# microsoft/XPretrain

Hardware: NVIDIA H100
Metric: video-text pairs/sec (12f x 224^2, 32 tok), CLIP-ViP ViT-B/16 fwd+InfoNCE+bwd (higher is better)
Workload: dtype bf16

## Files before the change

### xpretrain_b200/csrc/ptx.cuh

```cuda
#pragma once
#include <cuda.h>
#include <cuda_bf16.h>
#include <cuda_runtime.h>
#include <stdint.h>
#include <stdio.h>

namespace xp {

#ifndef XP_WAIT_TIMEOUT_CYCLES
#define XP_WAIT_TIMEOUT_CYCLES (8000000000ll)
#endif

__device__ __forceinline__ uint32_t smem_u32(const void* p) {
  return static_cast<uint32_t>(__cvta_generic_to_shared(p));
}
__device__ __forceinline__ int lane_id() { return threadIdx.x & 31; }

__device__ __forceinline__ void mbar_init(uint64_t* bar, uint32_t count) {
  asm volatile("mbarrier.init.shared::cta.b64 [%0], %1;" ::"r"(smem_u32(bar)), "r"(count) : "memory");
}
__device__ __forceinline__ void fence_barrier_init() {
  asm volatile("fence.mbarrier_init.release.cluster;" ::: "memory");
}
__device__ __forceinline__ void fence_proxy_async_smem() {
  asm volatile("fence.proxy.async.shared::cta;" ::: "memory");
}
__device__ __forceinline__ void mbar_arrive_expect_tx(uint64_t* bar, uint32_t bytes) {
  asm volatile("mbarrier.arrive.expect_tx.shared::cta.b64 _, [%0], %1;" ::"r"(smem_u32(bar)), "r"(bytes)
               : "memory");
}
__device__ __forceinline__ void mbar_arrive(uint64_t* bar) {
  asm volatile("mbarrier.arrive.shared::cta.b64 _, [%0];" ::"r"(smem_u32(bar)) : "memory");
}
__device__ __forceinline__ bool mbar_try_wait(uint64_t* bar, uint32_t parity) {
  uint32_t ok;
  asm volatile(
      "{\n"
      ".reg .pred p;\n"
      "mbarrier.try_wait.parity.shared::cta.b64 p, [%1], %2;\n"
      "selp.u32 %0, 1, 0, p;\n"
      "}\n"
      : "=r"(ok)
      : "r"(smem_u32(bar)), "r"(parity)
      : "memory");
  return ok != 0;
}
__device__ __forceinline__ void mbar_wait(uint64_t* bar, uint32_t parity) {
  if (mbar_try_wait(bar, parity)) return;
  long long t0 = clock64();
  while (!mbar_try_wait(bar, parity)) {
    if (clock64() - t0 > XP_WAIT_TIMEOUT_CYCLES) {
      printf("xpretrain_b200: mbarrier wait timeout (block %d thread %d parity %u)\n", blockIdx.x, threadIdx.x,
             parity);
      __trap();
    }
  }
}
__device__ __forceinline__ void mbar_wait_nocall(uint64_t* bar, uint32_t parity) {
  if (mbar_try_wait(bar, parity)) return;
  long long t0 = clock64();
  while (!mbar_try_wait(bar, parity)) {
    if (clock64() - t0 > XP_WAIT_TIMEOUT_CYCLES) __trap();
  }
}

__device__ __forceinline__ void tma_prefetch_desc(const CUtensorMap* m) {
  asm volatile("prefetch.tensormap [%0];" ::"l"(reinterpret_cast<uint64_t>(m)) : "memory");
}
__device__ __forceinline__ void tma_load_2d(void* smem_dst, const CUtensorMap* m, uint64_t* bar, int c0, int c1) {
  asm volatile(
      "cp.async.bulk.tensor.2d.shared::cluster.global.mbarrier::complete_tx::bytes [%0], [%1, {%3, %4}], [%2];"
      ::"r"(smem_u32(smem_dst)), "l"(reinterpret_cast<uint64_t>(m)), "r"(smem_u32(bar)), "r"(c0), "r"(c1)
      : "memory");
}
__device__ __forceinline__ void tma_load_3d(void* smem_dst, const CUtensorMap* m, uint64_t* bar, int c0, int c1,
                                            int c2) {
  asm volatile(
      "cp.async.bulk.tensor.3d.shared::cluster.global.mbarrier::complete_tx::bytes [%0], [%1, {%3, %4, %5}], [%2];"
      ::"r"(smem_u32(smem_dst)), "l"(reinterpret_cast<uint64_t>(m)), "r"(smem_u32(bar)), "r"(c0), "r"(c1), "r"(c2)
      : "memory");
}

__device__ __forceinline__ void tma_store_2d(const CUtensorMap* m, uint32_t smem_src, int c0, int c1) {
  asm volatile("cp.async.bulk.tensor.2d.global.shared::cta.bulk_group [%0, {%2, %3}], [%1];" ::"l"(
                   reinterpret_cast<uint64_t>(m)),
               "r"(smem_src), "r"(c0), "r"(c1)
               : "memory");
}
__device__ __forceinline__ void tma_store_commit() { asm volatile("cp.async.bulk.commit_group;" ::: "memory"); }
template <int N>
__device__ __forceinline__ void tma_store_wait_read() {
  asm volatile("cp.async.bulk.wait_group.read %0;" ::"n"(N) : "memory");
}

__device__ __forceinline__ void wgmma_fence() { asm volatile("wgmma.fence.sync.aligned;" ::: "memory"); }
__device__ __forceinline__ void wgmma_commit() { asm volatile("wgmma.commit_group.sync.aligned;" ::: "memory"); }
template <int N>
__device__ __forceinline__ void wgmma_wait() {
  asm volatile("wgmma.wait_group.sync.aligned %0;" ::"n"(N) : "memory");
}
template <int R>
__device__ __forceinline__ void wgmma_fence_regs(float (&d)[R]) {
#pragma unroll
  for (int i = 0; i < R; ++i) asm volatile("" : "+f"(d[i])::"memory");
}

template <int TA, int TB>
__device__ __forceinline__ void wgmma_m64n128k16_bf16(float (&d)[64], uint64_t adesc, uint64_t bdesc) {
  asm volatile(
      "wgmma.mma_async.sync.aligned.m64n128k16.f32.bf16.bf16 {"
      "%0, %1, %2, %3, %4, %5, %6, %7, %8, %9, %10, %11, %12, %13, %14, %15, "
      "%16, %17, %18, %19, %20, %21, %22, %23, %24, %25, %26, %27, %28, %29, %30, %31, "
      "%32, %33, %34, %35, %36, %37, %38, %39, %40, %41, %42, %43, %44, %45, %46, %47, "
      "%48, %49, %50, %51, %52, %53, %54, %55, %56, %57, %58, %59, %60, %61, %62, %63"
      "}, %64, %65, 1, 1, 1, %66, %67;"
      : "+f"(d[0]), "+f"(d[1]), "+f"(d[2]), "+f"(d[3]), "+f"(d[4]), "+f"(d[5]), "+f"(d[6]), "+f"(d[7]),
        "+f"(d[8]), "+f"(d[9]), "+f"(d[10]), "+f"(d[11]), "+f"(d[12]), "+f"(d[13]), "+f"(d[14]), "+f"(d[15]),
        "+f"(d[16]), "+f"(d[17]), "+f"(d[18]), "+f"(d[19]), "+f"(d[20]), "+f"(d[21]), "+f"(d[22]), "+f"(d[23]),
        "+f"(d[24]), "+f"(d[25]), "+f"(d[26]), "+f"(d[27]), "+f"(d[28]), "+f"(d[29]), "+f"(d[30]), "+f"(d[31]),
        "+f"(d[32]), "+f"(d[33]), "+f"(d[34]), "+f"(d[35]), "+f"(d[36]), "+f"(d[37]), "+f"(d[38]), "+f"(d[39]),
        "+f"(d[40]), "+f"(d[41]), "+f"(d[42]), "+f"(d[43]), "+f"(d[44]), "+f"(d[45]), "+f"(d[46]), "+f"(d[47]),
        "+f"(d[48]), "+f"(d[49]), "+f"(d[50]), "+f"(d[51]), "+f"(d[52]), "+f"(d[53]), "+f"(d[54]), "+f"(d[55]),
        "+f"(d[56]), "+f"(d[57]), "+f"(d[58]), "+f"(d[59]), "+f"(d[60]), "+f"(d[61]), "+f"(d[62]), "+f"(d[63])
      : "l"(adesc), "l"(bdesc), "n"(TA), "n"(TB));
}

template <int TA, int TB>
__device__ __forceinline__ void wgmma_m64n64k16_ss(float (&d)[32], uint64_t adesc, uint64_t bdesc) {
  asm volatile(
      "wgmma.mma_async.sync.aligned.m64n64k16.f32.bf16.bf16 {"
      "%0, %1, %2, %3, %4, %5, %6, %7, %8, %9, %10, %11, %12, %13, %14, %15, "
      "%16, %17, %18, %19, %20, %21, %22, %23, %24, %25, %26, %27, %28, %29, %30, %31"
      "}, %32, %33, 1, 1, 1, %34, %35;"
      : "+f"(d[0]), "+f"(d[1]), "+f"(d[2]), "+f"(d[3]), "+f"(d[4]), "+f"(d[5]), "+f"(d[6]), "+f"(d[7]),
        "+f"(d[8]), "+f"(d[9]), "+f"(d[10]), "+f"(d[11]), "+f"(d[12]), "+f"(d[13]), "+f"(d[14]), "+f"(d[15]),
        "+f"(d[16]), "+f"(d[17]), "+f"(d[18]), "+f"(d[19]), "+f"(d[20]), "+f"(d[21]), "+f"(d[22]), "+f"(d[23]),
        "+f"(d[24]), "+f"(d[25]), "+f"(d[26]), "+f"(d[27]), "+f"(d[28]), "+f"(d[29]), "+f"(d[30]), "+f"(d[31])
      : "l"(adesc), "l"(bdesc), "n"(TA), "n"(TB));
}
template <int TB>
__device__ __forceinline__ void wgmma_m64n64k16_rs(float (&d)[32], const uint32_t (&a)[4], uint64_t bdesc) {
  asm volatile(
      "wgmma.mma_async.sync.aligned.m64n64k16.f32.bf16.bf16 {"
      "%0, %1, %2, %3, %4, %5, %6, %7, %8, %9, %10, %11, %12, %13, %14, %15, "
      "%16, %17, %18, %19, %20, %21, %22, %23, %24, %25, %26, %27, %28, %29, %30, %31"
      "}, {%32, %33, %34, %35}, %36, 1, 1, 1, %37;"
      : "+f"(d[0]), "+f"(d[1]), "+f"(d[2]), "+f"(d[3]), "+f"(d[4]), "+f"(d[5]), "+f"(d[6]), "+f"(d[7]),
        "+f"(d[8]), "+f"(d[9]), "+f"(d[10]), "+f"(d[11]), "+f"(d[12]), "+f"(d[13]), "+f"(d[14]), "+f"(d[15]),
        "+f"(d[16]), "+f"(d[17]), "+f"(d[18]), "+f"(d[19]), "+f"(d[20]), "+f"(d[21]), "+f"(d[22]), "+f"(d[23]),
        "+f"(d[24]), "+f"(d[25]), "+f"(d[26]), "+f"(d[27]), "+f"(d[28]), "+f"(d[29]), "+f"(d[30]), "+f"(d[31])
      : "r"(a[0]), "r"(a[1]), "r"(a[2]), "r"(a[3]), "l"(bdesc), "n"(TB));
}

template <uint32_t N>
__device__ __forceinline__ void setmaxnreg_dec() {
  asm volatile("setmaxnreg.dec.sync.aligned.u32 %0;" ::"n"(N));
}
template <uint32_t N>
__device__ __forceinline__ void setmaxnreg_inc() {
  asm volatile("setmaxnreg.inc.sync.aligned.u32 %0;" ::"n"(N));
}
__device__ __forceinline__ void named_bar_sync(uint32_t id, uint32_t threads) {
  asm volatile("bar.sync %0, %1;" ::"r"(id), "r"(threads) : "memory");
}
__device__ __forceinline__ void named_bar_arrive(uint32_t id, uint32_t threads) {
  asm volatile("bar.arrive %0, %1;" ::"r"(id), "r"(threads) : "memory");
}

__device__ __forceinline__ uint64_t make_smem_desc_sw128(uint32_t smem_addr, uint32_t lbo_bytes,
                                                         uint32_t sbo_bytes) {
  uint64_t d = 0;
  d |= static_cast<uint64_t>((smem_addr & 0x3FFFF) >> 4);
  d |= static_cast<uint64_t>((lbo_bytes >> 4) & 0x3FFF) << 16;
  d |= static_cast<uint64_t>((sbo_bytes >> 4) & 0x3FFF) << 32;
  d |= static_cast<uint64_t>(1) << 62;
  return d;
}

__device__ __forceinline__ void quad_transpose(uint32_t (&v)[4]) {
  const int q = threadIdx.x & 3;
  uint32_t out[4];
  out[0] = out[1] = out[2] = out[3] = 0u;
#pragma unroll
  for (int t = 0; t < 4; ++t) {
    const int j = q ^ t;
    const uint32_t send = j == 0 ? v[0] : j == 1 ? v[1] : j == 2 ? v[2] : v[3];
    const uint32_t got = t == 0 ? send : __shfl_xor_sync(0xffffffffu, send, t);
#pragma unroll
    for (int c = 0; c < 4; ++c)
      if (c == j) out[c] = got;
  }
#pragma unroll
  for (int c = 0; c < 4; ++c) v[c] = out[c];
}

__device__ __forceinline__ uint32_t pack_bf16(float lo, float hi) {
  __nv_bfloat162 v = __floats2bfloat162_rn(lo, hi);
  return *reinterpret_cast<uint32_t*>(&v);
}
__device__ __forceinline__ float bf16_lo(uint32_t v) { return __uint_as_float(v << 16); }
__device__ __forceinline__ float bf16_hi(uint32_t v) { return __uint_as_float(v & 0xFFFF0000u); }

__device__ __forceinline__ float fast_sigmoid(float y) {
  float t;
  asm("tanh.approx.f32 %0, %1;" : "=f"(t) : "f"(0.5f * y));
  return fmaf(0.5f, t, 0.5f);
}
__device__ __forceinline__ float quick_gelu(float x) { return x * fast_sigmoid(1.702f * x); }
__device__ __forceinline__ float quick_gelu_grad(float x) {
  float y = 1.702f * x;
  y = y > 64.f ? 64.f : (y < -64.f ? -64.f : y);
  const float s = fast_sigmoid(y);
  return s * fmaf(y, 1.f - s, 1.f);
}

}
```

### xpretrain_b200/csrc/vip_attention.cu

```cuda
#include "../../include/xpretrain_b200.h"
#include "common.h"
#include "ptx.cuh"
#include "mma_frag.cuh"
#include "vip_attention.h"

namespace xp {

constexpr int SROWS = 256;
constexpr int GROW = 248;
constexpr int MAT_BYTES = SROWS * 128;
constexpr int TILE_BYTES = 64 * 128;
constexpr int ATT_THREADS = 256;

__device__ __forceinline__ bool row_valid(int r, const AttnDims& d) { return r < d.L || (r >= GROW && r < GROW + d.M); }
__device__ __forceinline__ bool row_global(int r) { return r >= GROW; }
__device__ __forceinline__ int row_seq(int r, const AttnDims& d) { return r >= GROW ? r - GROW : d.M + r; }
__device__ __forceinline__ bool tile_live(int k, const AttnDims& d) { return k == 3 || 64 * k < d.L; }

__device__ __forceinline__ uint64_t kdesc(uint32_t addr) { return make_smem_desc_sw128(addr, 16, 1024); }
__device__ __forceinline__ uint64_t mndesc(uint32_t addr) { return make_smem_desc_sw128(addr, 8192, 1024); }

template <int NMAT>
__device__ __forceinline__ void stage_rows(uint8_t* sm, uint64_t* bar, const CUtensorMap* const (&mapL)[NMAT],
                                           const CUtensorMap* const (&mapM)[NMAT], const int (&col)[NMAT], const AttnDims& d,
                                           int b, int t) {
  if (threadIdx.x == 0) {
    mbar_init(bar, 1);
    fence_barrier_init();
  }
  const uint32_t base = smem_u32(sm);
  for (int idx = threadIdx.x; idx < NMAT * SROWS * 8; idx += ATT_THREADS) {
    const int m = idx / (SROWS * 8), row = (idx >> 3) % SROWS;
    if (!row_valid(row, d)) st_shared_zero16(base + m * MAT_BYTES + row * 128 + (idx & 7) * 16);
  }
  fence_proxy_async_smem();
  __syncthreads();
  if (threadIdx.x == 0) {
    mbar_arrive_expect_tx(bar, NMAT * (d.L + d.M) * 128);
#pragma unroll
    for (int m = 0; m < NMAT; ++m) {
      tma_load_2d(sm + m * MAT_BYTES, mapL[m], bar, col[m], static_cast<int>(b * d.S + d.M + static_cast<long long>(t) * d.L));
      tma_load_2d(sm + m * MAT_BYTES + GROW * 128, mapM[m], bar, col[m], static_cast<int>(b * d.S));
    }
  }
  mbar_wait_nocall(bar, 0);
}

__device__ __forceinline__ void acc_to_afrag(const float (&x)[32], uint32_t (&a)[4][4]) {
#pragma unroll
  for (int ks = 0; ks < 4; ++ks) {
    a[ks][0] = pack_bf16(x[8 * ks + 0], x[8 * ks + 1]);
    a[ks][1] = pack_bf16(x[8 * ks + 2], x[8 * ks + 3]);
    a[ks][2] = pack_bf16(x[8 * ks + 4], x[8 * ks + 5]);
    a[ks][3] = pack_bf16(x[8 * ks + 6], x[8 * ks + 7]);
  }
}

__global__ void __launch_bounds__(ATT_THREADS, 2)
vip_attn_fwd_kernel(const __grid_constant__ CUtensorMap tmL, const __grid_constant__ CUtensorMap tmM,
                    __nv_bfloat16* __restrict__ out, float* __restrict__ lse, float* __restrict__ part, const AttnDims d) {
  extern __shared__ uint8_t smem_raw[];
  uint8_t* sm = smem_raw + (((smem_u32(smem_raw) + 1023u) & ~1023u) - smem_u32(smem_raw));
  uint64_t* bar = reinterpret_cast<uint64_t*>(sm + 3 * MAT_BYTES);
  const int t = blockIdx.x, h = blockIdx.y, b = blockIdx.z;
  {
    const CUtensorMap* const mL[3] = {&tmL, &tmL, &tmL};
    const CUtensorMap* const mM[3] = {&tmM, &tmM, &tmM};
    const int col[3] = {h * HD, d.C + h * HD, 2 * d.C + h * HD};
    stage_rows<3>(sm, bar, mL, mM, col, d, b, t);
  }
  const uint32_t sQ = smem_u32(sm), sK = sQ + MAT_BYTES, sV = sK + MAT_BYTES;
  const int wg = threadIdx.x >> 7, wq = (threadIdx.x >> 5) & 3, lane = threadIdx.x & 31;
  const bool mask_gg = (t != 0);

  for (int qt = wg; qt < 4; qt += 2) {
    if (!tile_live(qt, d)) continue;
    const int r_lo = qt * 64 + wq * 16 + (lane >> 2);
    const bool qg[2] = {row_global(r_lo), row_global(r_lo + 8)};
    float o[32];
#pragma unroll
    for (int i = 0; i < 32; ++i) o[i] = 0.f;
    float m_run[2] = {-INFINITY, -INFINITY}, l_run[2] = {0.f, 0.f};
#pragma unroll 1
    for (int kb = 0; kb < 4; ++kb) {
      if (!tile_live(kb, d)) continue;
      float s[32];
#pragma unroll
      for (int i = 0; i < 32; ++i) s[i] = 0.f;
      wgmma_fence_regs(s);
      wgmma_fence();
#pragma unroll
      for (int ks = 0; ks < 4; ++ks)
        wgmma_m64n64k16_ss<0, 0>(s, kdesc(sQ + qt * TILE_BYTES + ks * 32), kdesc(sK + kb * TILE_BYTES + ks * 32));
      wgmma_commit();
      wgmma_wait<0>();
      wgmma_fence_regs(s);
      float mx[2] = {-INFINITY, -INFINITY};
#pragma unroll
      for (int i = 0; i < 8; ++i)
#pragma unroll
        for (int e = 0; e < 4; ++e) {
          const int key = kb * 64 + i * 8 + (lane & 3) * 2 + (e & 1);
          const bool dead = !row_valid(key, d) || (mask_gg && qg[e >> 1] && row_global(key));
          if (dead) s[4 * i + e] = -INFINITY;
          mx[e >> 1] = fmaxf(mx[e >> 1], s[4 * i + e]);
        }
      float corr[2], mb[2];
#pragma unroll
      for (int r = 0; r < 2; ++r) {
        mx[r] = fmaxf(mx[r], __shfl_xor_sync(0xffffffffu, mx[r], 1));
        mx[r] = fmaxf(mx[r], __shfl_xor_sync(0xffffffffu, mx[r], 2));
        const float m_new = fmaxf(m_run[r], mx[r]);
        corr[r] = (m_new == -INFINITY) ? 1.f : fast_exp2((m_run[r] - m_new) * LOG2E);
        l_run[r] *= corr[r];
        m_run[r] = m_new;
        mb[r] = m_new == -INFINITY ? 0.f : m_new * LOG2E;
      }
#pragma unroll
      for (int i = 0; i < 8; ++i) {
        o[4 * i + 0] *= corr[0]; o[4 * i + 1] *= corr[0];
        o[4 * i + 2] *= corr[1]; o[4 * i + 3] *= corr[1];
      }
#pragma unroll
      for (int i = 0; i < 32; ++i) {
        const float pv = fast_exp2(fmaf(s[i], LOG2E, -mb[(i >> 1) & 1]));
        s[i] = pv;
        l_run[(i >> 1) & 1] += pv;
      }
      uint32_t ph[4][4], pl[4][4];
      acc_to_afrag(s, ph);
#pragma unroll
      for (int ks = 0; ks < 4; ++ks)
#pragma unroll
        for (int j = 0; j < 4; ++j)
          pl[ks][j] = pack_bf16(s[8 * ks + 2 * j] - bf16_lo(ph[ks][j]), s[8 * ks + 2 * j + 1] - bf16_hi(ph[ks][j]));
      wgmma_fence_regs(o);
      wgmma_fence();
#pragma unroll
      for (int ks = 0; ks < 4; ++ks) {
        const uint64_t vd = mndesc(sV + kb * TILE_BYTES + ks * 16 * 128);
        wgmma_m64n64k16_rs<1>(o, ph[ks], vd);
        wgmma_m64n64k16_rs<1>(o, pl[ks], vd);
      }
      wgmma_commit();
      wgmma_wait<0>();
      wgmma_fence_regs(o);
    }
#pragma unroll
    for (int r = 0; r < 2; ++r) {
      l_run[r] += __shfl_xor_sync(0xffffffffu, l_run[r], 1);
      l_run[r] += __shfl_xor_sync(0xffffffffu, l_run[r], 2);
    }
#pragma unroll
    for (int r = 0; r < 2; ++r) {
      const int row = r_lo + r * 8;
      if (!row_valid(row, d)) continue;
      if (row_global(row)) {
        float* p = part + (((static_cast<long long>(b) * d.H + h) * d.T + t) * d.M + (row - GROW)) * 66;
        if ((lane & 3) == 0) {
          p[0] = m_run[r];
          p[1] = l_run[r];
        }
#pragma unroll
        for (int i = 0; i < 8; ++i) {
          p[2 + i * 8 + (lane & 3) * 2] = o[4 * i + 2 * r];
          p[2 + i * 8 + (lane & 3) * 2 + 1] = o[4 * i + 2 * r + 1];
        }
      } else {
        const float inv = l_run[r] > 0.f ? 1.f / l_run[r] : 0.f;
        const long long tr = token_row(d, b, t, row_seq(row, d));
        __nv_bfloat16* dst = out + tr * d.ld_o + h * HD + (lane & 3) * 2;
#pragma unroll
        for (int i = 0; i < 8; ++i)
          *reinterpret_cast<uint32_t*>(dst + i * 8) = pack_bf16(o[4 * i + 2 * r] * inv, o[4 * i + 2 * r + 1] * inv);
        if ((lane & 3) == 0)
          lse[(static_cast<long long>(b) * d.H + h) * d.S + (tr - static_cast<long long>(b) * d.S)] = m_run[r] + logf(l_run[r]);
      }
    }
  }
}

__global__ void __launch_bounds__(64)
vip_attn_fwd_combine_kernel(const float* __restrict__ part, __nv_bfloat16* __restrict__ out, float* __restrict__ lse,
                            const AttnDims d) {
  const int h = blockIdx.x, b = blockIdx.y, c = threadIdx.x;
  for (int m = 0; m < d.M; ++m) {
    const float* p0 = part + ((static_cast<long long>(b) * d.H + h) * d.T * d.M + m) * 66;
    float mx = -INFINITY;
    for (int t = 0; t < d.T; ++t) mx = fmaxf(mx, p0[static_cast<long long>(t) * d.M * 66]);
    float l = 0.f, acc = 0.f;
    for (int t = 0; t < d.T; ++t) {
      const float* p = p0 + static_cast<long long>(t) * d.M * 66;
      const float w = __expf(p[0] - mx);
      l += p[1] * w;
      acc += p[2 + c] * w;
    }
    out[(static_cast<long long>(b) * d.S + m) * d.ld_o + h * HD + c] = __float2bfloat16(acc / l);
    if (c == 0) lse[(static_cast<long long>(b) * d.H + h) * d.S + m] = mx + logf(l);
  }
}


__global__ void __launch_bounds__(ATT_THREADS, 1)
vip_attn_bwd_kernel(const __grid_constant__ CUtensorMap tmL, const __grid_constant__ CUtensorMap tmM,
                    const __grid_constant__ CUtensorMap tdL, const __grid_constant__ CUtensorMap tdM,
                    const __nv_bfloat16* __restrict__ out, const __nv_bfloat16* __restrict__ dout, const float* __restrict__ lse,
                    __nv_bfloat16* __restrict__ dqkv, float* __restrict__ gpart, const AttnDims d, float q_scale) {
  extern __shared__ uint8_t smem_raw[];
  uint8_t* sm = smem_raw + (((smem_u32(smem_raw) + 1023u) & ~1023u) - smem_u32(smem_raw));
  float* s_lse = reinterpret_cast<float*>(sm + 4 * MAT_BYTES);
  float* s_delta = s_lse + SROWS;
  uint64_t* bar = reinterpret_cast<uint64_t*>(s_delta + SROWS);
  const int t = blockIdx.x, h = blockIdx.y, b = blockIdx.z;
  {
    const CUtensorMap* const mL[4] = {&tmL, &tmL, &tmL, &tdL};
    const CUtensorMap* const mM[4] = {&tmM, &tmM, &tmM, &tdM};
    const int col[4] = {h * HD, d.C + h * HD, 2 * d.C + h * HD, h * HD};
    stage_rows<4>(sm, bar, mL, mM, col, d, b, t);
  }
  for (int base = 0; base < SROWS; base += ATT_THREADS / 8) {
    const int row = base + (threadIdx.x >> 3), chunk = threadIdx.x & 7;
    float dot = 0.f;
    const bool valid = row_valid(row, d);
    long long tr = 0;
    if (valid) {
      tr = token_row(d, b, t, row_seq(row, d));
      const long long off = tr * d.ld_o + h * HD + chunk * 8;
      const uint4 g = *reinterpret_cast<const uint4*>(dout + off);
      const uint4 o = *reinterpret_cast<const uint4*>(out + off);
      const uint32_t gw[4] = {g.x, g.y, g.z, g.w}, ow[4] = {o.x, o.y, o.z, o.w};
#pragma unroll
      for (int i = 0; i < 4; ++i) dot += bf16_lo(gw[i]) * bf16_lo(ow[i]) + bf16_hi(gw[i]) * bf16_hi(ow[i]);
    }
    dot += __shfl_xor_sync(0xffffffffu, dot, 1);
    dot += __shfl_xor_sync(0xffffffffu, dot, 2);
    dot += __shfl_xor_sync(0xffffffffu, dot, 4);
    if (chunk == 0) {
      s_delta[row] = dot;
      s_lse[row] = valid ? lse[(static_cast<long long>(b) * d.H + h) * d.S + (tr - static_cast<long long>(b) * d.S)] * LOG2E
                         : INFINITY;
    }
  }
  __syncthreads();

  const uint32_t sQ = smem_u32(sm), sK = sQ + MAT_BYTES, sV = sK + MAT_BYTES, sdO = sV + MAT_BYTES;
  const int wg = threadIdx.x >> 7, wq = (threadIdx.x >> 5) & 3, lane = threadIdx.x & 31;
  const bool mask_gg = (t != 0);
  float* gp = gpart + ((static_cast<long long>(b) * d.H + h) * d.T + t) * d.M * 3 * HD;

  for (int kt = wg; kt < 4; kt += 2) {
    if (!tile_live(kt, d)) continue;
    const int k_lo = kt * 64 + wq * 16 + (lane >> 2);
    float dk[32], dv[32];
#pragma unroll
    for (int i = 0; i < 32; ++i) dk[i] = dv[i] = 0.f;
#pragma unroll 1
    for (int qb = 0; qb < 4; ++qb) {
      if (!tile_live(qb, d)) continue;
      float st[32], dpt[32];
#pragma unroll
      for (int i = 0; i < 32; ++i) st[i] = dpt[i] = 0.f;
      wgmma_fence_regs(st);
      wgmma_fence_regs(dpt);
      wgmma_fence();
#pragma unroll
      for (int ks = 0; ks < 4; ++ks) {
        wgmma_m64n64k16_ss<0, 0>(st, kdesc(sK + kt * TILE_BYTES + ks * 32), kdesc(sQ + qb * TILE_BYTES + ks * 32));
        wgmma_m64n64k16_ss<0, 0>(dpt, kdesc(sV + kt * TILE_BYTES + ks * 32), kdesc(sdO + qb * TILE_BYTES + ks * 32));
      }
      wgmma_commit();
      wgmma_wait<0>();
      wgmma_fence_regs(st);
      wgmma_fence_regs(dpt);
#pragma unroll
      for (int i = 0; i < 8; ++i)
#pragma unroll
        for (int e = 0; e < 4; ++e) {
          const int q = qb * 64 + i * 8 + (lane & 3) * 2 + (e & 1);
          const int key = k_lo + (e >> 1) * 8;
          const bool valid = row_valid(q, d) && row_valid(key, d) && !(mask_gg && row_global(q) && row_global(key));
          const float p = valid ? fast_exp2(fmaf(st[4 * i + e], LOG2E, -s_lse[q])) : 0.f;
          st[4 * i + e] = p;
          dpt[4 * i + e] = p * (dpt[4 * i + e] - s_delta[q]);
        }
      uint32_t ap[4][4], ad[4][4];
      acc_to_afrag(st, ap);
      acc_to_afrag(dpt, ad);
      wgmma_fence_regs(dv);
      wgmma_fence_regs(dk);
      wgmma_fence();
#pragma unroll
      for (int ks = 0; ks < 4; ++ks) {
        wgmma_m64n64k16_rs<1>(dv, ap[ks], mndesc(sdO + qb * TILE_BYTES + ks * 16 * 128));
        wgmma_m64n64k16_rs<1>(dk, ad[ks], mndesc(sQ + qb * TILE_BYTES + ks * 16 * 128));
      }
      wgmma_commit();
      wgmma_wait<0>();
      wgmma_fence_regs(dv);
      wgmma_fence_regs(dk);
    }
#pragma unroll
    for (int r = 0; r < 2; ++r) {
      const int key = k_lo + r * 8;
      if (!row_valid(key, d)) continue;
      if (!row_global(key)) {
        __nv_bfloat16* row = dqkv + token_row(d, b, t, row_seq(key, d)) * d.ld_qkv + h * HD + (lane & 3) * 2;
#pragma unroll
        for (int i = 0; i < 8; ++i) {
          *reinterpret_cast<uint32_t*>(row + d.C + i * 8) = pack_bf16(dk[4 * i + 2 * r], dk[4 * i + 2 * r + 1]);
          *reinterpret_cast<uint32_t*>(row + 2 * d.C + i * 8) = pack_bf16(dv[4 * i + 2 * r], dv[4 * i + 2 * r + 1]);
        }
      } else {
        float* g = gp + static_cast<long long>(key - GROW) * 3 * HD + (lane & 3) * 2;
#pragma unroll
        for (int i = 0; i < 8; ++i) {
          g[HD + i * 8] = dk[4 * i + 2 * r]; g[HD + i * 8 + 1] = dk[4 * i + 2 * r + 1];
          g[2 * HD + i * 8] = dv[4 * i + 2 * r]; g[2 * HD + i * 8 + 1] = dv[4 * i + 2 * r + 1];
        }
      }
    }
  }

  for (int qt = wg; qt < 4; qt += 2) {
    if (!tile_live(qt, d)) continue;
    const int q_lo = qt * 64 + wq * 16 + (lane >> 2);
    const float lse_r[2] = {s_lse[q_lo], s_lse[q_lo + 8]}, del_r[2] = {s_delta[q_lo], s_delta[q_lo + 8]};
    float dq[32];
#pragma unroll
    for (int i = 0; i < 32; ++i) dq[i] = 0.f;
#pragma unroll 1
    for (int kb = 0; kb < 4; ++kb) {
      if (!tile_live(kb, d)) continue;
      float s[32], dp[32];
#pragma unroll
      for (int i = 0; i < 32; ++i) s[i] = dp[i] = 0.f;
      wgmma_fence_regs(s);
      wgmma_fence_regs(dp);
      wgmma_fence();
#pragma unroll
      for (int ks = 0; ks < 4; ++ks) {
        wgmma_m64n64k16_ss<0, 0>(s, kdesc(sQ + qt * TILE_BYTES + ks * 32), kdesc(sK + kb * TILE_BYTES + ks * 32));
        wgmma_m64n64k16_ss<0, 0>(dp, kdesc(sdO + qt * TILE_BYTES + ks * 32), kdesc(sV + kb * TILE_BYTES + ks * 32));
      }
      wgmma_commit();
      wgmma_wait<0>();
      wgmma_fence_regs(s);
      wgmma_fence_regs(dp);
#pragma unroll
      for (int i = 0; i < 8; ++i)
#pragma unroll
        for (int e = 0; e < 4; ++e) {
          const int key = kb * 64 + i * 8 + (lane & 3) * 2 + (e & 1);
          const int q = q_lo + (e >> 1) * 8;
          const bool valid = row_valid(q, d) && row_valid(key, d) && !(mask_gg && row_global(q) && row_global(key));
          const float p = valid ? fast_exp2(fmaf(s[4 * i + e], LOG2E, -lse_r[e >> 1])) : 0.f;
          dp[4 * i + e] = p * (dp[4 * i + e] - del_r[e >> 1]);
        }
      uint32_t ad[4][4];
      acc_to_afrag(dp, ad);
      wgmma_fence_regs(dq);
      wgmma_fence();
#pragma unroll
      for (int ks = 0; ks < 4; ++ks) wgmma_m64n64k16_rs<1>(dq, ad[ks], mndesc(sK + kb * TILE_BYTES + ks * 16 * 128));
      wgmma_commit();
      wgmma_wait<0>();
      wgmma_fence_regs(dq);
    }
#pragma unroll
    for (int r = 0; r < 2; ++r) {
      const int q = q_lo + r * 8;
      if (!row_valid(q, d)) continue;
      if (!row_global(q)) {
        __nv_bfloat16* row = dqkv + token_row(d, b, t, row_seq(q, d)) * d.ld_qkv + h * HD + (lane & 3) * 2;
#pragma unroll
        for (int i = 0; i < 8; ++i)
          *reinterpret_cast<uint32_t*>(row + i * 8) = pack_bf16(dq[4 * i + 2 * r] * q_scale, dq[4 * i + 2 * r + 1] * q_scale);
      } else {
        float* g = gp + static_cast<long long>(q - GROW) * 3 * HD + (lane & 3) * 2;
#pragma unroll
        for (int i = 0; i < 8; ++i) {
          g[i * 8] = dq[4 * i + 2 * r];
          g[i * 8 + 1] = dq[4 * i + 2 * r + 1];
        }
      }
    }
  }
}

__global__ void __launch_bounds__(192)
vip_attn_bwd_combine_kernel(const float* __restrict__ gpart, __nv_bfloat16* __restrict__ dqkv, const AttnDims d,
                            float q_scale) {
  const int h = blockIdx.x, b = blockIdx.y;
  const int which = threadIdx.x / HD, c = threadIdx.x % HD;
  for (int m = 0; m < d.M; ++m) {
    float acc = 0.f;
    for (int t = 0; t < d.T; ++t)
      acc += gpart[((((static_cast<long long>(b) * d.H + h) * d.T + t) * d.M + m) * 3 + which) * HD + c];
    if (which == 0) acc *= q_scale;
    dqkv[(static_cast<long long>(b) * d.S + m) * d.ld_qkv + static_cast<long long>(which) * d.C + h * HD + c] =
        __float2bfloat16(acc);
  }
}


static int make_dims(AttnDims& d, int B, int H, int T, int L, int M, int C) {
  if (C != H * HD) return fail("vip_attention: head_dim must be 64 (C == 64*H)");
  if (L < 1) return fail("vip_attention: L must be >= 1");
  if (M < 1 || M > 8) return fail("vip_attention: 1 <= M <= 8 global tokens");
  d.B = B; d.H = H; d.T = T; d.L = L; d.M = M;
  d.S = static_cast<long long>(M) + static_cast<long long>(T) * L;
  d.C = C;
  d.ld_qkv = 3LL * C;
  d.ld_o = C;
  return 0;
}

static int make_row_maps(CUtensorMap* mL, CUtensorMap* mM, const void* base, long long width, const AttnDims& d) {
  const uint64_t rows = static_cast<uint64_t>(d.B) * static_cast<uint64_t>(d.S);
  if (make_tmap_bf16_2d(mL, base, width, rows, width, HD, d.L)) return -1;
  return make_tmap_bf16_2d(mM, base, width, rows, width, HD, d.M);
}

constexpr int FWD_SMEM = 3 * MAT_BYTES + 1024 + 64;
constexpr int BWD_SMEM = 4 * MAT_BYTES + 2 * SROWS * 4 + 1024 + 64;

}

using namespace xp;

extern "C" int64_t xp_vip_attention_workspace_bytes(int32_t B, int32_t H, int32_t T, int32_t M) {
  return static_cast<int64_t>(B) * H * T * M * 3 * HD * sizeof(float);
}

extern "C" int xp_vip_attention_fwd(const void* qkv, void* out, float* lse, float* workspace, int32_t B, int32_t H,
                                    int32_t T, int32_t L, int32_t M, int32_t C, void* stream) {
  XP_ENTER(qkv);
  AttnDims d;
  if (make_dims(d, B, H, T, L, M, C)) return -1;
  cudaStream_t st = static_cast<cudaStream_t>(stream);
  if (M + L > VIP_STAGED_MAX_ROWS) {
    if (vip_long_attn_fwd(d, qkv, out, lse, workspace, st)) return -1;
  } else {
    CUtensorMap mL, mM;
    if (make_row_maps(&mL, &mM, qkv, 3LL * C, d)) return -1;
    static bool attr = false;
    if (!attr) {
      XP_CHECK_CUDA(cudaFuncSetAttribute(vip_attn_fwd_kernel, cudaFuncAttributeMaxDynamicSharedMemorySize, FWD_SMEM));
      attr = true;
    }
    vip_attn_fwd_kernel<<<dim3(T, H, B), ATT_THREADS, FWD_SMEM, st>>>(mL, mM, static_cast<__nv_bfloat16*>(out), lse, workspace, d);
    XP_CHECK_LAUNCH("vip_attn_fwd_kernel");
  }
  vip_attn_fwd_combine_kernel<<<dim3(H, B), 64, 0, st>>>(workspace, static_cast<__nv_bfloat16*>(out), lse, d);
  XP_CHECK_LAUNCH("vip_attn_fwd_combine_kernel");
  return 0;
}

extern "C" int xp_vip_attention_bwd(const void* qkv, const void* out, const void* dout, const float* lse, void* dqkv,
                                    float* workspace, int32_t B, int32_t H, int32_t T, int32_t L, int32_t M, int32_t C,
                                    float q_scale, void* stream) {
  XP_ENTER(qkv);
  AttnDims d;
  if (make_dims(d, B, H, T, L, M, C)) return -1;
  cudaStream_t st = static_cast<cudaStream_t>(stream);
  if (M + L > VIP_STAGED_MAX_ROWS) {
    if (vip_long_attn_bwd(d, qkv, out, dout, lse, dqkv, workspace, q_scale, st)) return -1;
  } else {
    CUtensorMap mL, mM, gL, gM;
    if (make_row_maps(&mL, &mM, qkv, 3LL * C, d) || make_row_maps(&gL, &gM, dout, C, d)) return -1;
    static bool attr = false;
    if (!attr) {
      XP_CHECK_CUDA(cudaFuncSetAttribute(vip_attn_bwd_kernel, cudaFuncAttributeMaxDynamicSharedMemorySize, BWD_SMEM));
      attr = true;
    }
    vip_attn_bwd_kernel<<<dim3(T, H, B), ATT_THREADS, BWD_SMEM, st>>>(
        mL, mM, gL, gM, static_cast<const __nv_bfloat16*>(out), static_cast<const __nv_bfloat16*>(dout), lse,
        static_cast<__nv_bfloat16*>(dqkv), workspace, d, q_scale);
    XP_CHECK_LAUNCH("vip_attn_bwd_kernel");
  }
  vip_attn_bwd_combine_kernel<<<dim3(H, B), 192, 0, st>>>(workspace, static_cast<__nv_bfloat16*>(dqkv), d, q_scale);
  XP_CHECK_LAUNCH("vip_attn_bwd_combine_kernel");
  return 0;
}
```

Baseline: 245.6.

## Size attention staging to actual frame length and reuse dS panels for dQ

Replaces the fixed 256-row staging layout with a Stage struct sized to L rounded up to 16 plus the global tokens. Edge key blocks dispatch to narrower wgmma shapes (n16/32/48) so padded rows are not computed, and masking is applied only on edge blocks. The backward pass stores dS panels in shared memory during the dK/dV loop, then computes dQ as one panel-times-K GEMM instead of recomputing S and dP. Shared memory use now varies per launch, which may change occupancy, and the added panel storage and synchronisation make the kernel more complex.

```diff
diff --git a/xpretrain_b200/csrc/ptx.cuh b/xpretrain_b200/csrc/ptx.cuh
--- a/xpretrain_b200/csrc/ptx.cuh
+++ b/xpretrain_b200/csrc/ptx.cuh
@@ -138,6 +138,45 @@
         "+f"(d[24]), "+f"(d[25]), "+f"(d[26]), "+f"(d[27]), "+f"(d[28]), "+f"(d[29]), "+f"(d[30]), "+f"(d[31])
       : "l"(adesc), "l"(bdesc), "n"(TA), "n"(TB));
 }
+template <int TA, int TB>
+__device__ __forceinline__ void wgmma_m64n48k16_ss(float (&d)[24], uint64_t adesc, uint64_t bdesc) {
+  asm volatile(
+      "wgmma.mma_async.sync.aligned.m64n48k16.f32.bf16.bf16 {"
+      "%0, %1, %2, %3, %4, %5, %6, %7, %8, %9, %10, %11, %12, %13, %14, %15, "
+      "%16, %17, %18, %19, %20, %21, %22, %23"
+      "}, %24, %25, 1, 1, 1, %26, %27;"
+      : "+f"(d[0]), "+f"(d[1]), "+f"(d[2]), "+f"(d[3]), "+f"(d[4]), "+f"(d[5]), "+f"(d[6]), "+f"(d[7]),
+        "+f"(d[8]), "+f"(d[9]), "+f"(d[10]), "+f"(d[11]), "+f"(d[12]), "+f"(d[13]), "+f"(d[14]), "+f"(d[15]),
+        "+f"(d[16]), "+f"(d[17]), "+f"(d[18]), "+f"(d[19]), "+f"(d[20]), "+f"(d[21]), "+f"(d[22]), "+f"(d[23])
+      : "l"(adesc), "l"(bdesc), "n"(TA), "n"(TB));
+}
+template <int TA, int TB>
+__device__ __forceinline__ void wgmma_m64n32k16_ss(float (&d)[16], uint64_t adesc, uint64_t bdesc) {
+  asm volatile(
+      "wgmma.mma_async.sync.aligned.m64n32k16.f32.bf16.bf16 {"
+      "%0, %1, %2, %3, %4, %5, %6, %7, %8, %9, %10, %11, %12, %13, %14, %15"
+      "}, %16, %17, 1, 1, 1, %18, %19;"
+      : "+f"(d[0]), "+f"(d[1]), "+f"(d[2]), "+f"(d[3]), "+f"(d[4]), "+f"(d[5]), "+f"(d[6]), "+f"(d[7]),
+        "+f"(d[8]), "+f"(d[9]), "+f"(d[10]), "+f"(d[11]), "+f"(d[12]), "+f"(d[13]), "+f"(d[14]), "+f"(d[15])
+      : "l"(adesc), "l"(bdesc), "n"(TA), "n"(TB));
+}
+template <int TA, int TB>
+__device__ __forceinline__ void wgmma_m64n16k16_ss(float (&d)[8], uint64_t adesc, uint64_t bdesc) {
+  asm volatile(
+      "wgmma.mma_async.sync.aligned.m64n16k16.f32.bf16.bf16 {"
+      "%0, %1, %2, %3, %4, %5, %6, %7"
+      "}, %8, %9, 1, 1, 1, %10, %11;"
+      : "+f"(d[0]), "+f"(d[1]), "+f"(d[2]), "+f"(d[3]), "+f"(d[4]), "+f"(d[5]), "+f"(d[6]), "+f"(d[7])
+      : "l"(adesc), "l"(bdesc), "n"(TA), "n"(TB));
+}
+template <int N, int TA, int TB>
+__device__ __forceinline__ void wgmma_m64nNk16_ss(float (&d)[N / 2], uint64_t adesc, uint64_t bdesc) {
+  static_assert(N == 16 || N == 32 || N == 48 || N == 64, "wgmma N");
+  if constexpr (N == 64) wgmma_m64n64k16_ss<TA, TB>(d, adesc, bdesc);
+  else if constexpr (N == 48) wgmma_m64n48k16_ss<TA, TB>(d, adesc, bdesc);
+  else if constexpr (N == 32) wgmma_m64n32k16_ss<TA, TB>(d, adesc, bdesc);
+  else wgmma_m64n16k16_ss<TA, TB>(d, adesc, bdesc);
+}
 template <int TB>
 __device__ __forceinline__ void wgmma_m64n64k16_rs(float (&d)[32], const uint32_t (&a)[4], uint64_t bdesc) {
   asm volatile(
diff --git a/xpretrain_b200/csrc/vip_attention.cu b/xpretrain_b200/csrc/vip_attention.cu
--- a/xpretrain_b200/csrc/vip_attention.cu
+++ b/xpretrain_b200/csrc/vip_attention.cu
@@ -6,16 +6,20 @@
 
 namespace xp {
 
-constexpr int SROWS = 256;
-constexpr int GROW = 248;
-constexpr int MAT_BYTES = SROWS * 128;
 constexpr int TILE_BYTES = 64 * 128;
 constexpr int ATT_THREADS = 256;
-
-__device__ __forceinline__ bool row_valid(int r, const AttnDims& d) { return r < d.L || (r >= GROW && r < GROW + d.M); }
-__device__ __forceinline__ bool row_global(int r) { return r >= GROW; }
-__device__ __forceinline__ int row_seq(int r, const AttnDims& d) { return r >= GROW ? r - GROW : d.M + r; }
-__device__ __forceinline__ bool tile_live(int k, const AttnDims& d) { return k == 3 || 64 * k < d.L; }
+constexpr int MAX_STAGE_ROWS = 224;
+
+struct Stage {
+  int L, M, G, R;
+  __host__ __device__ Stage(int L_, int M_) : L(L_), M(M_), G(((L_ + 15) & ~15) + 8), R(((L_ + 15) & ~15) + 16) {}
+  __host__ __device__ int tiles() const { return (R + 63) / 64; }
+  __host__ __device__ int mat_bytes() const { return R * 128; }
+  __device__ bool valid(int r) const { return r < L || (r >= G && r < G + M); }
+  __device__ bool global(int r) const { return r >= G && r < G + M; }
+  __device__ int seq(int r) const { return r >= G ? r - G : M + r; }
+  __device__ bool edge(int blk) const { return 64 * blk + 64 > L; }
+};
 
 __device__ __forceinline__ uint64_t kdesc(uint32_t addr) { return make_smem_desc_sw128(addr, 16, 1024); }
 __device__ __forceinline__ uint64_t mndesc(uint32_t addr) { return make_smem_desc_sw128(addr, 8192, 1024); }
@@ -23,15 +27,17 @@
 template <int NMAT>
 __device__ __forceinline__ void stage_rows(uint8_t* sm, uint64_t* bar, const CUtensorMap* const (&mapL)[NMAT],
                                            const CUtensorMap* const (&mapM)[NMAT], const int (&col)[NMAT], const AttnDims& d,
-                                           int b, int t) {
+                                           const Stage& sg, int b, int t) {
   if (threadIdx.x == 0) {
     mbar_init(bar, 1);
     fence_barrier_init();
   }
   const uint32_t base = smem_u32(sm);
-  for (int idx = threadIdx.x; idx < NMAT * SROWS * 8; idx += ATT_THREADS) {
-    const int m = idx / (SROWS * 8), row = (idx >> 3) % SROWS;
-    if (!row_valid(row, d)) st_shared_zero16(base + m * MAT_BYTES + row * 128 + (idx & 7) * 16);
+  const int gap = sg.G - sg.L, nzero = sg.R - sg.L - sg.M;
+  for (int idx = threadIdx.x; idx < NMAT * nzero * 8; idx += ATT_THREADS) {
+    const int m = idx / (nzero * 8), j = (idx >> 3) % nzero;
+    const int row = j < gap ? sg.L + j : sg.M + sg.L + j;
+    st_shared_zero16(base + m * sg.mat_bytes() + row * 128 + (idx & 7) * 16);
   }
   fence_proxy_async_smem();
   __syncthreads();
@@ -39,112 +45,135 @@
     mbar_arrive_expect_tx(bar, NMAT * (d.L + d.M) * 128);
 #pragma unroll
     for (int m = 0; m < NMAT; ++m) {
-      tma_load_2d(sm + m * MAT_BYTES, mapL[m], bar, col[m], static_cast<int>(b * d.S + d.M + static_cast<long long>(t) * d.L));
-      tma_load_2d(sm + m * MAT_BYTES + GROW * 128, mapM[m], bar, col[m], static_cast<int>(b * d.S));
-    }
-  }
-  mbar_wait_nocall(bar, 0);
-}
-
-__device__ __forceinline__ void acc_to_afrag(const float (&x)[32], uint32_t (&a)[4][4]) {
-#pragma unroll
-  for (int ks = 0; ks < 4; ++ks) {
+      uint8_t* dst = sm + m * sg.mat_bytes();
+      tma_load_2d(dst, mapL[m], bar, col[m], static_cast<int>(b * d.S + d.M + static_cast<long long>(t) * d.L));
+      tma_load_2d(dst + sg.G * 128, mapM[m], bar, col[m], static_cast<int>(b * d.S));
+    }
+  }
+}
+
+template <int NW>
+__device__ __forceinline__ void acc_to_afrag(const float (&x)[NW / 2], uint32_t (&a)[NW / 16][4]) {
+#pragma unroll
+  for (int ks = 0; ks < NW / 16; ++ks) {
     a[ks][0] = pack_bf16(x[8 * ks + 0], x[8 * ks + 1]);
     a[ks][1] = pack_bf16(x[8 * ks + 2], x[8 * ks + 3]);
     a[ks][2] = pack_bf16(x[8 * ks + 4], x[8 * ks + 5]);
     a[ks][3] = pack_bf16(x[8 * ks + 6], x[8 * ks + 7]);
   }
 }
+
+template <int NW, bool MASK>
+__device__ __forceinline__ void fwd_block(float (&o)[32], float (&m_run)[2], float (&l_run)[2], uint32_t sQ_tile,
+                                          uint32_t sK_blk, uint32_t sV_blk, int key0, const Stage& sg, bool mask_gg,
+                                          const bool (&qg)[2], int lane) {
+  float s[NW / 2];
+#pragma unroll
+  for (int i = 0; i < NW / 2; ++i) s[i] = 0.f;
+  wgmma_fence_regs(s);
+  wgmma_fence();
+#pragma unroll
+  for (int ks = 0; ks < 4; ++ks) wgmma_m64nNk16_ss<NW, 0, 0>(s, kdesc(sQ_tile + ks * 32), kdesc(sK_blk + ks * 32));
+  wgmma_commit();
+  wgmma_wait<0>();
+  wgmma_fence_regs(s);
+  float mx[2] = {-INFINITY, -INFINITY};
+#pragma unroll
+  for (int i = 0; i < NW / 8; ++i)
+#pragma unroll
+    for (int e = 0; e < 4; ++e) {
+      if constexpr (MASK) {
+        const int key = key0 + i * 8 + (lane & 3) * 2 + (e & 1);
+        const bool dead = !sg.valid(key) || (mask_gg && qg[e >> 1] && sg.global(key));
+        s[4 * i + e] = dead ? -INFINITY : s[4 * i + e];
+      }
+      mx[e >> 1] = fmaxf(mx[e >> 1], s[4 * i + e]);
+    }
+  float corr[2], mb[2];
+#pragma unroll
+  for (int r = 0; r < 2; ++r) {
+    mx[r] = fmaxf(mx[r], __shfl_xor_sync(0xffffffffu, mx[r], 1));
+    mx[r] = fmaxf(mx[r], __shfl_xor_sync(0xffffffffu, mx[r], 2));
+    const float m_new = fmaxf(m_run[r], mx[r]);
+    corr[r] = (m_new == -INFINITY) ? 1.f : fast_exp2((m_run[r] - m_new) * LOG2E);
+    l_run[r] *= corr[r];
+    m_run[r] = m_new;
+    mb[r] = m_new == -INFINITY ? 0.f : m_new * LOG2E;
+  }
+#pragma unroll
+  for (int i = 0; i < 8; ++i) {
+    o[4 * i + 0] *= corr[0]; o[4 * i + 1] *= corr[0];
+    o[4 * i + 2] *= corr[1]; o[4 * i + 3] *= corr[1];
+  }
+#pragma unroll
+  for (int i = 0; i < NW / 2; ++i) {
+    const float pv = fast_exp2(fmaf(s[i], LOG2E, -mb[(i >> 1) & 1]));
+    s[i] = pv;
+    l_run[(i >> 1) & 1] += pv;
+  }
+  uint32_t ph[NW / 16][4], pl[NW / 16][4];
+  acc_to_afrag<NW>(s, ph);
+#pragma unroll
+  for (int ks = 0; ks < NW / 16; ++ks)
+#pragma unroll
+    for (int j = 0; j < 4; ++j)
+      pl[ks][j] = pack_bf16(s[8 * ks + 2 * j] - bf16_lo(ph[ks][j]), s[8 * ks + 2 * j + 1] - bf16_hi(ph[ks][j]));
+  wgmma_fence_regs(o);
+  wgmma_fence();
+#pragma unroll
+  for (int ks = 0; ks < NW / 16; ++ks) {
+    const uint64_t vd = mndesc(sV_blk + ks * 16 * 128);
+    wgmma_m64n64k16_rs<1>(o, ph[ks], vd);
+    wgmma_m64n64k16_rs<1>(o, pl[ks], vd);
+  }
+  wgmma_commit();
+  wgmma_wait<0>();
+  wgmma_fence_regs(o);
+}
+
+__host__ __device__ constexpr int fwd_mats_bytes(int R) { return (3 * R > 64 * ((R + 63) / 64) ? 3 * R : 64 * ((R + 63) / 64)) * 128; }
 
 __global__ void __launch_bounds__(ATT_THREADS, 2)
 vip_attn_fwd_kernel(const __grid_constant__ CUtensorMap tmL, const __grid_constant__ CUtensorMap tmM,
                     __nv_bfloat16* __restrict__ out, float* __restrict__ lse, float* __restrict__ part, const AttnDims d) {
   extern __shared__ uint8_t smem_raw[];
   uint8_t* sm = smem_raw + (((smem_u32(smem_raw) + 1023u) & ~1023u) - smem_u32(smem_raw));
-  uint64_t* bar = reinterpret_cast<uint64_t*>(sm + 3 * MAT_BYTES);
+  const Stage sg(d.L, d.M);
+  uint64_t* bar = reinterpret_cast<uint64_t*>(sm + fwd_mats_bytes(sg.R));
   const int t = blockIdx.x, h = blockIdx.y, b = blockIdx.z;
   {
     const CUtensorMap* const mL[3] = {&tmL, &tmL, &tmL};
     const CUtensorMap* const mM[3] = {&tmM, &tmM, &tmM};
     const int col[3] = {h * HD, d.C + h * HD, 2 * d.C + h * HD};
-    stage_rows<3>(sm, bar, mL, mM, col, d, b, t);
-  }
-  const uint32_t sQ = smem_u32(sm), sK = sQ + MAT_BYTES, sV = sK + MAT_BYTES;
+    stage_rows<3>(sm, bar, mL, mM, col, d, sg, b, t);
+  }
+  mbar_wait_nocall(bar, 0);
+  const uint32_t sQ = smem_u32(sm), sK = sQ + sg.mat_bytes(), sV = sK + sg.mat_bytes();
   const int wg = threadIdx.x >> 7, wq = (threadIdx.x >> 5) & 3, lane = threadIdx.x & 31;
   const bool mask_gg = (t != 0);
-
-  for (int qt = wg; qt < 4; qt += 2) {
-    if (!tile_live(qt, d)) continue;
+  const int nt = sg.tiles();
+
+  for (int qt = wg; qt < nt; qt += 2) {
     const int r_lo = qt * 64 + wq * 16 + (lane >> 2);
-    const bool qg[2] = {row_global(r_lo), row_global(r_lo + 8)};
+    const bool qg[2] = {sg.global(r_lo), sg.global(r_lo + 8)};
     float o[32];
 #pragma unroll
     for (int i = 0; i < 32; ++i) o[i] = 0.f;
     float m_run[2] = {-INFINITY, -INFINITY}, l_run[2] = {0.f, 0.f};
+    const uint32_t sQ_tile = sQ + qt * TILE_BYTES;
 #pragma unroll 1
-    for (int kb = 0; kb < 4; ++kb) {
-      if (!tile_live(kb, d)) continue;
-      float s[32];
-#pragma unroll
-      for (int i = 0; i < 32; ++i) s[i] = 0.f;
-      wgmma_fence_regs(s);
-      wgmma_fence();
-#pragma unroll
-      for (int ks = 0; ks < 4; ++ks)
-        wgmma_m64n64k16_ss<0, 0>(s, kdesc(sQ + qt * TILE_BYTES + ks * 32), kdesc(sK + kb * TILE_BYTES + ks * 32));
-      wgmma_commit();
-      wgmma_wait<0>();
-      wgmma_fence_regs(s);
-      float mx[2] = {-INFINITY, -INFINITY};
-#pragma unroll
-      for (int i = 0; i < 8; ++i)
-#pragma unroll
-        for (int e = 0; e < 4; ++e) {
-          const int key = kb * 64 + i * 8 + (lane & 3) * 2 + (e & 1);
-          const bool dead = !row_valid(key, d) || (mask_gg && qg[e >> 1] && row_global(key));
-          if (dead) s[4 * i + e] = -INFINITY;
-          mx[e >> 1] = fmaxf(mx[e >> 1], s[4 * i + e]);
-        }
-      float corr[2], mb[2];
-#pragma unroll
-      for (int r = 0; r < 2; ++r) {
-        mx[r] = fmaxf(mx[r], __shfl_xor_sync(0xffffffffu, mx[r], 1));
-        mx[r] = fmaxf(mx[r], __shfl_xor_sync(0xffffffffu, mx[r], 2));
-        const float m_new = fmaxf(m_run[r], mx[r]);
-        corr[r] = (m_new == -INFINITY) ? 1.f : fast_exp2((m_run[r] - m_new) * LOG2E);
-        l_run[r] *= corr[r];
-        m_run[r] = m_new;
-        mb[r] = m_new == -INFINITY ? 0.f : m_new * LOG2E;
-      }
-#pragma unroll
-      for (int i = 0; i < 8; ++i) {
-        o[4 * i + 0] *= corr[0]; o[4 * i + 1] *= corr[0];
-        o[4 * i + 2] *= corr[1]; o[4 * i + 3] *= corr[1];
-      }
-#pragma unroll
-      for (int i = 0; i < 32; ++i) {
-        const float pv = fast_exp2(fmaf(s[i], LOG2E, -mb[(i >> 1) & 1]));
-        s[i] = pv;
-        l_run[(i >> 1) & 1] += pv;
-      }
-      uint32_t ph[4][4], pl[4][4];
-      acc_to_afrag(s, ph);
-#pragma unroll
-      for (int ks = 0; ks < 4; ++ks)
-#pragma unroll
-        for (int j = 0; j < 4; ++j)
-          pl[ks][j] = pack_bf16(s[8 * ks + 2 * j] - bf16_lo(ph[ks][j]), s[8 * ks + 2 * j + 1] - bf16_hi(ph[ks][j]));
-      wgmma_fence_regs(o);
-      wgmma_fence();
-#pragma unroll
-      for (int ks = 0; ks < 4; ++ks) {
-        const uint64_t vd = mndesc(sV + kb * TILE_BYTES + ks * 16 * 128);
-        wgmma_m64n64k16_rs<1>(o, ph[ks], vd);
-        wgmma_m64n64k16_rs<1>(o, pl[ks], vd);
-      }
-      wgmma_commit();
-      wgmma_wait<0>();
-      wgmma_fence_regs(o);
+    for (int kb = 0; kb < nt; ++kb) {
+      const uint32_t sK_blk = sK + kb * TILE_BYTES, sV_blk = sV + kb * TILE_BYTES;
+      if (!sg.edge(kb)) {
+        fwd_block<64, false>(o, m_run, l_run, sQ_tile, sK_blk, sV_blk, kb * 64, sg, mask_gg, qg, lane);
+        continue;
+      }
+      switch (min(64, sg.R - 64 * kb)) {
+        case 16: fwd_block<16, true>(o, m_run, l_run, sQ_tile, sK_blk, sV_blk, kb * 64, sg, mask_gg, qg, lane); break;
+        case 32: fwd_block<32, true>(o, m_run, l_run, sQ_tile, sK_blk, sV_blk, kb * 64, sg, mask_gg, qg, lane); break;
+        case 48: fwd_block<48, true>(o, m_run, l_run, sQ_tile, sK_blk, sV_blk, kb * 64, sg, mask_gg, qg, lane); break;
+        default: fwd_block<64, true>(o, m_run, l_run, sQ_tile, sK_blk, sV_blk, kb * 64, sg, mask_gg, qg, lane); break;
+      }
     }
 #pragma unroll
     for (int r = 0; r < 2; ++r) {
@@ -154,9 +183,9 @@
 #pragma unroll
     for (int r = 0; r < 2; ++r) {
       const int row = r_lo + r * 8;
-      if (!row_valid(row, d)) continue;
-      if (row_global(row)) {
-        float* p = part + (((static_cast<long long>(b) * d.H + h) * d.T + t) * d.M + (row - GROW)) * 66;
+      if (!sg.valid(row)) continue;
+      if (sg.global(row)) {
+        float* p = part + (((static_cast<long long>(b) * d.H + h) * d.T + t) * d.M + (row - sg.G)) * 66;
         if ((lane & 3) == 0) {
           p[0] = m_run[r];
           p[1] = l_run[r];
@@ -168,7 +197,7 @@
         }
       } else {
         const float inv = l_run[r] > 0.f ? 1.f / l_run[r] : 0.f;
-        const long long tr = token_row(d, b, t, row_seq(row, d));
+        const long long tr = token_row(d, b, t, sg.seq(row));
         __nv_bfloat16* dst = out + tr * d.ld_o + h * HD + (lane & 3) * 2;
 #pragma unroll
         for (int i = 0; i < 8; ++i)
@@ -201,117 +230,183 @@
 }
 
 
+template <int NW, bool MASK>
+__device__ __forceinline__ void bwd_key_block(float (&dk)[32], float (&dv)[32], uint8_t* sm, uint32_t sK_tile,
+                                              uint32_t sV_tile, uint32_t sQ_blk, uint32_t sdO_blk, uint32_t panel_off,
+                                              const float* s_lse, const float* s_delta, int q0, int k_lo,
+                                              const Stage& sg, bool mask_gg, int lane) {
+  float st[NW / 2], dpt[NW / 2];
+#pragma unroll
+  for (int i = 0; i < NW / 2; ++i) st[i] = dpt[i] = 0.f;
+  wgmma_fence_regs(st);
+  wgmma_fence_regs(dpt);
+  wgmma_fence();
+#pragma unroll
+  for (int ks = 0; ks < 4; ++ks) {
+    wgmma_m64nNk16_ss<NW, 0, 0>(st, kdesc(sK_tile + ks * 32), kdesc(sQ_blk + ks * 32));
+    wgmma_m64nNk16_ss<NW, 0, 0>(dpt, kdesc(sV_tile + ks * 32), kdesc(sdO_blk + ks * 32));
+  }
+  wgmma_commit();
+  float2 lq[NW / 8], dq[NW / 8];
+#pragma unroll
+  for (int i = 0; i < NW / 8; ++i) {
+    lq[i] = *reinterpret_cast<const float2*>(s_lse + q0 + i * 8 + (lane & 3) * 2);
+    dq[i] = *reinterpret_cast<const float2*>(s_delta + q0 + i * 8 + (lane & 3) * 2);
+  }
+  wgmma_wait<0>();
+  wgmma_fence_regs(st);
+  wgmma_fence_regs(dpt);
+#pragma unroll
+  for (int i = 0; i < NW / 8; ++i)
+#pragma unroll
+    for (int e = 0; e < 4; ++e) {
+      const float l = (e & 1) ? lq[i].y : lq[i].x, dl = (e & 1) ? dq[i].y : dq[i].x;
+      const float p = fast_exp2(fmaf(st[4 * i + e], LOG2E, -l));
+      const float ds = p * (dpt[4 * i + e] - dl);
+      if constexpr (MASK) {
+        const int q = q0 + i * 8 + (lane & 3) * 2 + (e & 1);
+        const int key = k_lo + (e >> 1) * 8;
+        const bool valid = sg.valid(key) && !(mask_gg && sg.global(q) && sg.global(key));
+        st[4 * i + e] = valid ? p : 0.f;
+        dpt[4 * i + e] = valid ? ds : 0.f;
+      } else {
+        st[4 * i + e] = p;
+        dpt[4 * i + e] = ds;
+      }
+    }
+  uint32_t ap[NW / 16][4], ad[NW / 16][4];
+  acc_to_afrag<NW>(st, ap);
+  acc_to_afrag<NW>(dpt, ad);
+#pragma unroll
+  for (int ks = 0; ks < NW / 16; ++ks)
+#pragma unroll
+    for (int j = 0; j < 4; ++j) {
+      const int key = k_lo + (j & 1) * 8, chunk = 2 * ks + (j >> 1);
+      if (!MASK || key < sg.R)
+        *reinterpret_cast<uint32_t*>(sm + panel_off + key * 128 + ((chunk ^ (key & 7)) << 4) + (lane & 3) * 4) = ad[ks][j];
+    }
+  wgmma_fence_regs(dv);
+  wgmma_fence_regs(dk);
+  wgmma_fence();
+#pragma unroll
+  for (int ks = 0; ks < NW / 16; ++ks) {
+    wgmma_m64n64k16_rs<1>(dv, ap[ks], mndesc(sdO_blk + ks * 16 * 128));
+    wgmma_m64n64k16_rs<1>(dk, ad[ks], mndesc(sQ_blk + ks * 16 * 128));
+  }
+  wgmma_commit();
+  wgmma_wait<0>();
+  wgmma_fence_regs(dv);
+  wgmma_fence_regs(dk);
+}
+
+__host__ __device__ constexpr int bwd_smem_bytes(int R) { return (4 + (R + 63) / 64) * R * 128 + 2 * R * 4 + 1024 + 64; }
+
 __global__ void __launch_bounds__(ATT_THREADS, 1)
 vip_attn_bwd_kernel(const __grid_constant__ CUtensorMap tmL, const __grid_constant__ CUtensorMap tmM,
                     const __grid_constant__ CUtensorMap tdL, const __grid_constant__ CUtensorMap tdM,
-                    const __nv_bfloat16* __restrict__ out, const __nv_bfloat16* __restrict__ dout, const float* __restrict__ lse,
+                    const __nv_bfloat16* __restrict__ out, const float* __restrict__ lse,
                     __nv_bfloat16* __restrict__ dqkv, float* __restrict__ gpart, const AttnDims d, float q_scale) {
   extern __shared__ uint8_t smem_raw[];
   uint8_t* sm = smem_raw + (((smem_u32(smem_raw) + 1023u) & ~1023u) - smem_u32(smem_raw));
-  float* s_lse = reinterpret_cast<float*>(sm + 4 * MAT_BYTES);
-  float* s_delta = s_lse + SROWS;
-  uint64_t* bar = reinterpret_cast<uint64_t*>(s_delta + SROWS);
+  const Stage sg(d.L, d.M);
+  const int nt = sg.tiles(), mat = sg.mat_bytes();
+  const int panel0 = 4 * mat;
+  float* s_lse = reinterpret_cast<float*>(sm + (4 + nt) * mat);
+  float* s_delta = s_lse + sg.R;
+  uint64_t* bar = reinterpret_cast<uint64_t*>(s_delta + sg.R);
   const int t = blockIdx.x, h = blockIdx.y, b = blockIdx.z;
   {
     const CUtensorMap* const mL[4] = {&tmL, &tmL, &tmL, &tdL};
     const CUtensorMap* const mM[4] = {&tmM, &tmM, &tmM, &tdM};
-    const int col[4] = {h * HD, d.C + h * HD, 2 * d.C + h * HD, h * HD};
-    stage_rows<4>(sm, bar, mL, mM, col, d, b, t);
-  }
-  for (int base = 0; base < SROWS; base += ATT_THREADS / 8) {
-    const int row = base + (threadIdx.x >> 3), chunk = threadIdx.x & 7;
+    const int col[4] = {d.C + h * HD, 2 * d.C + h * HD, h * HD, h * HD};
+    stage_rows<4>(sm, bar, mL, mM, col, d, sg, b, t);
+  }
+  const uint32_t sK = smem_u32(sm), sV = sK + mat, sQ = sV + mat, sdO = sQ + mat;
+  constexpr int PRO_ITERS = MAX_STAGE_ROWS / (ATT_THREADS / 8);
+  const int chunk = threadIdx.x & 7;
+  uint4 o_pre[PRO_ITERS];
+  float lse_pre[PRO_ITERS];
+#pragma unroll
+  for (int j = 0; j < PRO_ITERS; ++j) {
+    const int row = j * (ATT_THREADS / 8) + (threadIdx.x >> 3);
+    o_pre[j] = make_uint4(0u, 0u, 0u, 0u);
+    lse_pre[j] = INFINITY;
+    if (row < sg.R && sg.valid(row)) {
+      const long long tr = token_row(d, b, t, sg.seq(row));
+      o_pre[j] = *reinterpret_cast<const uint4*>(out + tr * d.ld_o + h * HD + chunk * 8);
+      lse_pre[j] = lse[(static_cast<long long>(b) * d.H + h) * d.S + (tr - static_cast<long long>(b) * d.S)] * LOG2E;
+    }
+  }
+  mbar_wait_nocall(bar, 0);
+#pragma unroll
+  for (int j = 0; j < PRO_ITERS; ++j) {
+    const int row = j * (ATT_THREADS / 8) + (threadIdx.x >> 3);
     float dot = 0.f;
-    const bool valid = row_valid(row, d);
-    long long tr = 0;
-    if (valid) {
-      tr = token_row(d, b, t, row_seq(row, d));
-      const long long off = tr * d.ld_o + h * HD + chunk * 8;
-      const uint4 g = *reinterpret_cast<const uint4*>(dout + off);
-      const uint4 o = *reinterpret_cast<const uint4*>(out + off);
-      const uint32_t gw[4] = {g.x, g.y, g.z, g.w}, ow[4] = {o.x, o.y, o.z, o.w};
+    if (row < sg.R) {
+      const uint4 g = *reinterpret_cast<const uint4*>(sm + 3 * mat + row * 128 + ((chunk ^ (row & 7)) << 4));
+      const uint32_t gw[4] = {g.x, g.y, g.z, g.w}, ow[4] = {o_pre[j].x, o_pre[j].y, o_pre[j].z, o_pre[j].w};
 #pragma unroll
       for (int i = 0; i < 4; ++i) dot += bf16_lo(gw[i]) * bf16_lo(ow[i]) + bf16_hi(gw[i]) * bf16_hi(ow[i]);
     }
     dot += __shfl_xor_sync(0xffffffffu, dot, 1);
     dot += __shfl_xor_sync(0xffffffffu, dot, 2);
     dot += __shfl_xor_sync(0xffffffffu, dot, 4);
-    if (chunk == 0) {
+    if (chunk == 0 && row < sg.R) {
       s_delta[row] = dot;
-      s_lse[row] = valid ? lse[(static_cast<long long>(b) * d.H + h) * d.S + (tr - static_cast<long long>(b) * d.S)] * LOG2E
-                         : INFINITY;
+      s_lse[row] = lse_pre[j];
     }
   }
   __syncthreads();
 
-  const uint32_t sQ = smem_u32(sm), sK = sQ + MAT_BYTES, sV = sK + MAT_BYTES, sdO = sV + MAT_BYTES;
   const int wg = threadIdx.x >> 7, wq = (threadIdx.x >> 5) & 3, lane = threadIdx.x & 31;
   const bool mask_gg = (t != 0);
   float* gp = gpart + ((static_cast<long long>(b) * d.H + h) * d.T + t) * d.M * 3 * HD;
 
-  for (int kt = wg; kt < 4; kt += 2) {
-    if (!tile_live(kt, d)) continue;
+  if (wg == 0 && nt >= 2) named_bar_sync(1, ATT_THREADS);
+  for (int kt = wg; kt < nt; kt += 2) {
     const int k_lo = kt * 64 + wq * 16 + (lane >> 2);
+    const uint32_t sK_tile = sK + kt * TILE_BYTES, sV_tile = sV + kt * TILE_BYTES;
+    const bool edge = sg.edge(kt);
     float dk[32], dv[32];
 #pragma unroll
     for (int i = 0; i < 32; ++i) dk[i] = dv[i] = 0.f;
 #pragma unroll 1
-    for (int qb = 0; qb < 4; ++qb) {
-      if (!tile_live(qb, d)) continue;
-      float st[32], dpt[32];
-#pragma unroll
-      for (int i = 0; i < 32; ++i) st[i] = dpt[i] = 0.f;
-      wgmma_fence_regs(st);
-      wgmma_fence_regs(dpt);
-      wgmma_fence();
-#pragma unroll
-      for (int ks = 0; ks < 4; ++ks) {
-        wgmma_m64n64k16_ss<0, 0>(st, kdesc(sK + kt * TILE_BYTES + ks * 32), kdesc(sQ + qb * TILE_BYTES + ks * 32));
-        wgmma_m64n64k16_ss<0, 0>(dpt, kdesc(sV + kt * TILE_BYTES + ks * 32), kdesc(sdO + qb * TILE_BYTES + ks * 32));
-      }
-      wgmma_commit();
-      wgmma_wait<0>();
-      wgmma_fence_regs(st);
-      wgmma_fence_regs(dpt);
-#pragma unroll
-      for (int i = 0; i < 8; ++i)
-#pragma unroll
-        for (int e = 0; e < 4; ++e) {
-          const int q = qb * 64 + i * 8 + (lane & 3) * 2 + (e & 1);
-          const int key = k_lo + (e >> 1) * 8;
-          const bool valid = row_valid(q, d) && row_valid(key, d) && !(mask_gg && row_global(q) && row_global(key));
-          const float p = valid ? fast_exp2(fmaf(st[4 * i + e], LOG2E, -s_lse[q])) : 0.f;
-          st[4 * i + e] = p;
-          dpt[4 * i + e] = p * (dpt[4 * i + e] - s_delta[q]);
-        }
-      uint32_t ap[4][4], ad[4][4];
-      acc_to_afrag(st, ap);
-      acc_to_afrag(dpt, ad);
-      wgmma_fence_regs(dv);
-      wgmma_fence_regs(dk);
-      wgmma_fence();
-#pragma unroll
-      for (int ks = 0; ks < 4; ++ks) {
-        wgmma_m64n64k16_rs<1>(dv, ap[ks], mndesc(sdO + qb * TILE_BYTES + ks * 16 * 128));
-        wgmma_m64n64k16_rs<1>(dk, ad[ks], mndesc(sQ + qb * TILE_BYTES + ks * 16 * 128));
-      }
-      wgmma_commit();
-      wgmma_wait<0>();
-      wgmma_fence_regs(dv);
-      wgmma_fence_regs(dk);
+    for (int qb = 0; qb < nt; ++qb) {
+      const uint32_t sQ_blk = sQ + qb * TILE_BYTES, sdO_blk = sdO + qb * TILE_BYTES, panel = panel0 + qb * mat;
+      const int nw = min(64, sg.R - 64 * qb);
+#define XP_KEY_BLOCK(NW, MASK) \
+  bwd_key_block<NW, MASK>(dk, dv, sm, sK_tile, sV_tile, sQ_blk, sdO_blk, panel, s_lse, s_delta, qb * 64, k_lo, sg, mask_gg, lane)
+      if (edge) {
+        switch (nw) {
+          case 16: XP_KEY_BLOCK(16, true); break;
+          case 32: XP_KEY_BLOCK(32, true); break;
+          case 48: XP_KEY_BLOCK(48, true); break;
+          default: XP_KEY_BLOCK(64, true); break;
+        }
+      } else {
+        switch (nw) {
+          case 16: XP_KEY_BLOCK(16, false); break;
+          case 32: XP_KEY_BLOCK(32, false); break;
+          case 48: XP_KEY_BLOCK(48, false); break;
+          default: XP_KEY_BLOCK(64, false); break;
+        }
+      }
+#undef XP_KEY_BLOCK
+      if (wg == 1 && kt == 1 && qb == 0) named_bar_arrive(1, ATT_THREADS);
     }
 #pragma unroll
     for (int r = 0; r < 2; ++r) {
       const int key = k_lo + r * 8;
-      if (!row_valid(key, d)) continue;
-      if (!row_global(key)) {
-        __nv_bfloat16* row = dqkv + token_row(d, b, t, row_seq(key, d)) * d.ld_qkv + h * HD + (lane & 3) * 2;
+      if (!sg.valid(key)) continue;
+      if (!sg.global(key)) {
+        __nv_bfloat16* row = dqkv + token_row(d, b, t, sg.seq(key)) * d.ld_qkv + h * HD + (lane & 3) * 2;
 #pragma unroll
         for (int i = 0; i < 8; ++i) {
           *reinterpret_cast<uint32_t*>(row + d.C + i * 8) = pack_bf16(dk[4 * i + 2 * r], dk[4 * i + 2 * r + 1]);
           *reinterpret_cast<uint32_t*>(row + 2 * d.C + i * 8) = pack_bf16(dv[4 * i + 2 * r], dv[4 * i + 2 * r + 1]);
         }
       } else {
-        float* g = gp + static_cast<long long>(key - GROW) * 3 * HD + (lane & 3) * 2;
+        float* g = gp + static_cast<long long>(key - sg.G) * 3 * HD + (lane & 3) * 2;
 #pragma unroll
         for (int i = 0; i < 8; ++i) {
           g[HD + i * 8] = dk[4 * i + 2 * r]; g[HD + i * 8 + 1] = dk[4 * i + 2 * r + 1];
@@ -320,63 +415,34 @@
       }
     }
   }
-
-  for (int qt = wg; qt < 4; qt += 2) {
-    if (!tile_live(qt, d)) continue;
+  fence_proxy_async_smem();
+  __syncthreads();
+
+  for (int qt = wg; qt < nt; qt += 2) {
     const int q_lo = qt * 64 + wq * 16 + (lane >> 2);
-    const float lse_r[2] = {s_lse[q_lo], s_lse[q_lo + 8]}, del_r[2] = {s_delta[q_lo], s_delta[q_lo + 8]};
+    const uint32_t panel = smem_u32(sm) + panel0 + qt * mat;
     float dq[32];
 #pragma unroll
     for (int i = 0; i < 32; ++i) dq[i] = 0.f;
+    wgmma_fence_regs(dq);
+    wgmma_fence();
 #pragma unroll 1
-    for (int kb = 0; kb < 4; ++kb) {
-      if (!tile_live(kb, d)) continue;
-      float s[32], dp[32];
-#pragma unroll
-      for (int i = 0; i < 32; ++i) s[i] = dp[i] = 0.f;
-      wgmma_fence_regs(s);
-      wgmma_fence_regs(dp);
-      wgmma_fence();
-#pragma unroll
-      for (int ks = 0; ks < 4; ++ks) {
-        wgmma_m64n64k16_ss<0, 0>(s, kdesc(sQ + qt * TILE_BYTES + ks * 32), kdesc(sK + kb * TILE_BYTES + ks * 32));
-        wgmma_m64n64k16_ss<0, 0>(dp, kdesc(sdO + qt * TILE_BYTES + ks * 32), kdesc(sV + kb * TILE_BYTES + ks * 32));
-      }
-      wgmma_commit();
-      wgmma_wait<0>();
-      wgmma_fence_regs(s);
-      wgmma_fence_regs(dp);
-#pragma unroll
-      for (int i = 0; i < 8; ++i)
-#pragma unroll
-        for (int e = 0; e < 4; ++e) {
-          const int key = kb * 64 + i * 8 + (lane & 3) * 2 + (e & 1);
-          const int q = q_lo + (e >> 1) * 8;
-          const bool valid = row_valid(q, d) && row_valid(key, d) && !(mask_gg && row_global(q) && row_global(key));
-          const float p = valid ? fast_exp2(fmaf(s[4 * i + e], LOG2E, -lse_r[e >> 1])) : 0.f;
-          dp[4 * i + e] = p * (dp[4 * i + e] - del_r[e >> 1]);
-        }
-      uint32_t ad[4][4];
-      acc_to_afrag(dp, ad);
-      wgmma_fence_regs(dq);
-      wgmma_fence();
-#pragma unroll
-      for (int ks = 0; ks < 4; ++ks) wgmma_m64n64k16_rs<1>(dq, ad[ks], mndesc(sK + kb * TILE_BYTES + ks * 16 * 128));
-      wgmma_commit();
-      wgmma_wait<0>();
-      wgmma_fence_regs(dq);
-    }
+    for (int ks = 0; ks < sg.R / 16; ++ks)
+      wgmma_m64n64k16_ss<1, 1>(dq, mndesc(panel + ks * 16 * 128), mndesc(sK + ks * 16 * 128));
+    wgmma_commit();
+    wgmma_wait<0>();
+    wgmma_fence_regs(dq);
 #pragma unroll
     for (int r = 0; r < 2; ++r) {
       const int q = q_lo + r * 8;
-      if (!row_valid(q, d)) continue;
-      if (!row_global(q)) {
-        __nv_bfloat16* row = dqkv + token_row(d, b, t, row_seq(q, d)) * d.ld_qkv + h * HD + (lane & 3) * 2;
+      if (!sg.valid(q)) continue;
+      if (!sg.global(q)) {
+        __nv_bfloat16* row = dqkv + token_row(d, b, t, sg.seq(q)) * d.ld_qkv + h * HD + (lane & 3) * 2;
 #pragma unroll
         for (int i = 0; i < 8; ++i)
           *reinterpret_cast<uint32_t*>(row + i * 8) = pack_bf16(dq[4 * i + 2 * r] * q_scale, dq[4 * i + 2 * r + 1] * q_scale);
       } else {
-        float* g = gp + static_cast<long long>(q - GROW) * 3 * HD + (lane & 3) * 2;
+        float* g = gp + static_cast<long long>(q - sg.G) * 3 * HD + (lane & 3) * 2;
 #pragma unroll
         for (int i = 0; i < 8; ++i) {
           g[i * 8] = dq[4 * i + 2 * r];
@@ -421,8 +487,9 @@
   return make_tmap_bf16_2d(mM, base, width, rows, width, HD, d.M);
 }
 
-constexpr int FWD_SMEM = 3 * MAT_BYTES + 1024 + 64;
-constexpr int BWD_SMEM = 4 * MAT_BYTES + 2 * SROWS * 4 + 1024 + 64;
+constexpr int FWD_SMEM_MAX = fwd_mats_bytes(MAX_STAGE_ROWS) + 1024 + 64;
+constexpr int BWD_SMEM_MAX = bwd_smem_bytes(MAX_STAGE_ROWS);
+static_assert(BWD_SMEM_MAX <= 227 * 1024, "the backward's stage and dS panels exceed the opt-in shared memory");
 
 }
 
@@ -445,10 +512,11 @@
     if (make_row_maps(&mL, &mM, qkv, 3LL * C, d)) return -1;
     static bool attr = false;
     if (!attr) {
-      XP_CHECK_CUDA(cudaFuncSetAttribute(vip_attn_fwd_kernel, cudaFuncAttributeMaxDynamicSharedMemorySize, FWD_SMEM));
+      XP_CHECK_CUDA(cudaFuncSetAttribute(vip_attn_fwd_kernel, cudaFuncAttributeMaxDynamicSharedMemorySize, FWD_SMEM_MAX));
       attr = true;
     }
-    vip_attn_fwd_kernel<<<dim3(T, H, B), ATT_THREADS, FWD_SMEM, st>>>(mL, mM, static_cast<__nv_bfloat16*>(out), lse, workspace, d);
+    const int smem = fwd_mats_bytes(Stage(L, M).R) + 1024 + 64;
+    vip_attn_fwd_kernel<<<dim3(T, H, B), ATT_THREADS, smem, st>>>(mL, mM, static_cast<__nv_bfloat16*>(out), lse, workspace, d);
     XP_CHECK_LAUNCH("vip_attn_fwd_kernel");
   }
   vip_attn_fwd_combine_kernel<<<dim3(H, B), 64, 0, st>>>(workspace, static_cast<__nv_bfloat16*>(out), lse, d);
@@ -470,12 +538,12 @@
     if (make_row_maps(&mL, &mM, qkv, 3LL * C, d) || make_row_maps(&gL, &gM, dout, C, d)) return -1;
     static bool attr = false;
     if (!attr) {
-      XP_CHECK_CUDA(cudaFuncSetAttribute(vip_attn_bwd_kernel, cudaFuncAttributeMaxDynamicSharedMemorySize, BWD_SMEM));
+      XP_CHECK_CUDA(cudaFuncSetAttribute(vip_attn_bwd_kernel, cudaFuncAttributeMaxDynamicSharedMemorySize, BWD_SMEM_MAX));
       attr = true;
     }
-    vip_attn_bwd_kernel<<<dim3(T, H, B), ATT_THREADS, BWD_SMEM, st>>>(
-        mL, mM, gL, gM, static_cast<const __nv_bfloat16*>(out), static_cast<const __nv_bfloat16*>(dout), lse,
-        static_cast<__nv_bfloat16*>(dqkv), workspace, d, q_scale);
+    vip_attn_bwd_kernel<<<dim3(T, H, B), ATT_THREADS, bwd_smem_bytes(Stage(L, M).R), st>>>(
+        mL, mM, gL, gM, static_cast<const __nv_bfloat16*>(out), lse, static_cast<__nv_bfloat16*>(dqkv), workspace, d,
+        q_scale);
     XP_CHECK_LAUNCH("vip_attn_bwd_kernel");
   }
   vip_attn_bwd_combine_kernel<<<dim3(H, B), 192, 0, st>>>(workspace, static_cast<__nv_bfloat16*>(dqkv), d, q_scale);
```

Result: faster. 273.9, median of 6 (+11.5%).
